# lllyasviel/stable-diffusion-webui-forge

Hardware: AMD Instinct MI355X
Metric: sampler it/s (UNet steps/sec) (higher is better)
Workload: dtype f16; 1 GPU; SDXL UNet 1024x1024 batch=8/GPU fp16, Euler sampler, CFG 7.0 (network batch 16), HIP-graph replay=on; global_batch=8, parallelism=batch-shard x1 (RCCL broadcast cond + gather latents)

## Files before the change

stable-diffusion-webui-forge_amd/csrc/fmx_attention.hip:

```cpp
#include <stdlib.h>

#include "fmx_common.hpp"

namespace {

struct AttnParams {
  const f16* q;
  const f16* k;
  const f16* vt;
  f16* o;
  long q_bs, q_rs, k_bs, k_rs, vt_bs, vt_hs, vt_ds, o_bs, o_rs;
  int batch, heads, nq, nk, nk_pad, qtiles;
  float scale_log2e;
  int causal;
  const f16* zp;
  unsigned q_span;
  unsigned k_span, vt_span;
  const f16* mask;
  long mask_bs, mask_hs, mask_qs;
  float inv_scale;
  int nfull, nsplit;
  int bid0;
};

// ... 798 lines not shown
  const int wg = xcd_remap(blockIdx.x, p.nfull);
  const int qt = wg % p.qtiles, bh = wg / p.qtiles;
  const int h = bh % p.heads, b = bh / p.heads;
  const int q0 = qt * 256 + grp * 64;
  const int ntiles = (p.nk + KVB - 1) / KVB;
  char* const pbase = smem + OFF_P + grp * PSLOT;
  float* const lbase = reinterpret_cast<float*>(smem + OFF_L) + grp * 128;

  if (is_s) {
    const f16* kbase = p.k + (long)b * p.k_bs + (long)h * DP;
    const __amdgpu_buffer_rsrc_t rs_k = __builtin_amdgcn_make_buffer_rsrc(const_cast<f16*>(kbase), 0, p.k_span, 0x00020000);
    unsigned k_voff[NPK];
#pragma unroll
    for (int e = 0; e < NPK; ++e) {
      const int row = (e * 4 + grp) * KROWS + lane / CPR;
      k_voff[e] = (unsigned)row * (unsigned)p.k_rs * 2u + (unsigned)k_logical_chunk<CPR>(row, lane % CPR) * 16u;
    }
    const unsigned k_tile = (unsigned)KVB * (unsigned)p.k_rs * 2u;
    auto stage_k = [&](int slot, int kt) __attribute__((always_inline)) {
#pragma unroll
      for (int e = 0; e < NPK; ++e) {
        auto* dk = (__attribute__((address_space(3))) void*)(smem + slot * KBYTES + (e * 4 + grp) * 1024);
        const unsigned kv = k_voff[e];
        __builtin_amdgcn_raw_ptr_buffer_load_lds(rs_k, dk, 16, kv, (unsigned)kt * k_tile, 0, 0);
      }
    };
    stage_k(0, 0);
    if (ntiles > 1) stage_k(1, 1);
    const float c2 = p.scale_log2e;
    f16x8 qf[2][DSTEPS];
#pragma unroll
    for (int a = 0; a < 2; ++a) {
      const int qrow = min(q0 + a * 32 + li, p.nq - 1);
      const f16* qp = p.q + (long)b * p.q_bs + (long)qrow * p.q_rs + (long)h * DP + hi * 8;
#pragma unroll
      for (int ds = 0; ds < DSTEPS; ++ds) {
        const f16x8 raw = *reinterpret_cast<const f16x8*>(qp + ds * 16);
#pragma unroll
        for (int e = 0; e < 8; ++e) qf[a][ds][e] = (f16)((float)raw[e] * c2);
      }
    }
    float m_run[2] = {0.f, 0.f}, l_run[2] = {0.f, 0.f};
    f16x8 ones, mfrag[2];
#pragma unroll
    for (int e = 0; e < 8; ++e) {
      ones[e] = (f16)((hi == 0 && e < 2) ? 1.0f : 0.0f);
      mfrag[0][e] = mfrag[1][e] = (f16)0.0f;
    }
    const int krow = key_perm(li);
    wait_vmcnt0();
    __builtin_amdgcn_s_barrier();
    typedef unsigned u32x2 __attribute__((ext_vector_type(2)));
    f32x16 sacc[2][2];
    f16x8 kf[2][DSTEPS];
    auto read_k = [&](int which, const char* sk, int half) __attribute__((always_inline)) {
#pragma unroll
      for (int ds = 0; ds < DSTEPS; ++ds) {
        const int row = half * 32 + krow;
        kf[which][ds] = *reinterpret_cast<const f16x8*>(sk + row * (DP * 2) + (k_phys_chunk<CPR>(row, ds * 2 + hi) << 4));
      }
    };
    auto scores = [&](int which) __attribute__((always_inline)) {
#pragma unroll
      for (int a = 0; a < 2; ++a) {
        f32x16 z;
#pragma unroll
        for (int r = 0; r < 16; ++r) z[r] = 0.f;
        sacc[which][a] = FMX_MFMA_32x32x16(ones, mfrag[a], z);
      }
#pragma unroll
      for (int ds = 0; ds < DSTEPS; ++ds)
#pragma unroll
        for (int a = 0; a < 2; ++a) sacc[which][a] = FMX_MFMA_32x32x16(kf[which][ds], qf[a][ds], sacc[which][a]);
    };
    __builtin_amdgcn_sched_barrier(0);
    read_k(0, smem, 0);
    read_k(1, smem, 1);
    scores(0);
    __builtin_amdgcn_sched_barrier(0);
    int kslot_next = ntiles > 1 ? 1 : 0;
    for (int t = 0; t <= ntiles; ++t) {
      if (t < ntiles) {
        if (t + 2 < ntiles) stage_k(kslot_next == 2 ? 0 : kslot_next + 1, t + 2);
        const char* skn = smem + kslot_next * KBYTES;
        char* const ps = pbase + (t & 1) * (4 * PSLOT);
        float* const ctrl = reinterpret_cast<float*>(ps + 8 * 1024);
        const bool ragged = (t + 1) * KVB > p.nk;
#pragma unroll
        for (int s2 = 0; s2 < 2; ++s2) {
          __builtin_amdgcn_sched_barrier(0);
          if (ragged) {
#pragma unroll
            for (int a = 0; a < 2; ++a)
#pragma unroll
              for (int r = 0; r < 16; ++r)
                if (t * KVB + s2 * 32 + hi * 16 + r >= p.nk) sacc[s2][a][r] = -INFINITY;
          }
          float mx[2];
#pragma unroll
          for (int a = 0; a < 2; ++a) {
            float m0 = fmaxf(sacc[s2][a][0], sacc[s2][a][1]);
#pragma unroll
            for (int r = 2; r < 16; r += 2) m0 = fmaxf(fmaxf(m0, sacc[s2][a][r]), sacc[s2][a][r + 1]);
            const u32x2 sw = __builtin_amdgcn_permlane32_swap(__float_as_uint(m0), __float_as_uint(m0), false, false);
            mx[a] = fmaxf(__uint_as_float(sw[0]), __uint_as_float(sw[1]));
          }
          const bool first = t == 0 && s2 == 0;
          const bool moved = first || __any(fmaxf(mx[0], mx[1]) > (float)THR);
          if (moved) {
#pragma unroll
            for (int a = 0; a < 2; ++a) {
              const float delta = first ? mx[a] : fmaxf(mx[a], 0.f);
              const float alpha = first ? 1.0f : __builtin_amdgcn_exp2f(-delta);
              m_run[a] += delta;
              l_run[a] *= alpha;
              const f16 mh = (f16)(-m_run[a]);
              const f16 ml = (f16)(-m_run[a] - (float)mh);
              mfrag[a][0] = hi == 0 ? mh : (f16)0.0f;
              mfrag[a][1] = hi == 0 ? ml : (f16)0.0f;
              ctrl[(s2 * 2 + a) * 64 + lane] = alpha;
#pragma unroll
              for (int r = 0; r < 16; ++r) sacc[s2][a][r] -= delta;
            }
          }
          if (lane == 0) reinterpret_cast<int*>(ctrl)[256 + s2] = (moved && !first) ? 1 : 0;
          __builtin_amdgcn_sched_barrier(0);
          if (s2 == 0) {
            scores(1);
            read_k(0, skn, 0);
          } else {
            scores(0);
            read_k(1, skn, 1);
          }
#pragma unroll
          for (int a = 0; a < 2; ++a) {
            float ps0 = 0.f, ps1 = 0.f;
            f16x8 pf[2];
#pragma unroll
            for (int r = 0; r < 16; ++r) {
              const float e = __builtin_amdgcn_exp2f(sacc[s2][a][r]);
              if (r & 1) ps1 += e; else ps0 += e;
              pf[r >> 3][r & 7] = (f16)e;
            }
#pragma unroll
            for (int j = 0; j < 2; ++j) *reinterpret_cast<f16x8*>(ps + ((a * 2 + s2) * 2 + j) * 1024 + lane * 16) = pf[j];
            l_run[a] += ps0 + ps1;
          }
#pragma unroll
          for (int i = 0; i < 2 * DSTEPS + 2; ++i) {
            __builtin_amdgcn_sched_group_barrier(0x008, 1, 0);
            if (i < DSTEPS) __builtin_amdgcn_sched_group_barrier(0x100, 1, 0);
            __builtin_amdgcn_sched_group_barrier(0x402, (80 + DSTEPS) / (2 * DSTEPS + 2), 0);
          }
          __builtin_amdgcn_sched_barrier(0);
        }
        if (t + 1 == ntiles) {
          lbase[lane] = l_run[0];
          lbase[64 + lane] = l_run[1];
        }
        kslot_next = kslot_next == 2 ? 0 : kslot_next + 1;
      }
      asm volatile("s_waitcnt vmcnt(0) lgkmcnt(0)" ::: "memory");
      __builtin_amdgcn_s_barrier();
    }
    return;
  }

  const f16* vbase = p.vt + (long)b * p.vt_bs + (long)h * p.vt_hs;
  const __amdgpu_buffer_rsrc_t rs_v = __builtin_amdgcn_make_buffer_rsrc(const_cast<f16*>(vbase), 0, p.vt_span, 0x00020000);
  unsigned v_voff[NPV];
#pragma unroll
  for (int e = 0; e < NPV; ++e) {
    const int row = (e * 4 + grp) * 8 + (lane >> 3);
    v_voff[e] = (unsigned)row * (unsigned)p.vt_ds * 2u + (unsigned)((lane & 7) ^ ((row >> 1) & 7)) * 16u;
  }
  auto stage_v = [&](int slot, int kt) __attribute__((always_inline)) {
#pragma unroll
    for (int e = 0; e < NPV; ++e) {
      auto* dv = (__attribute__((address_space(3))) void*)(smem + OFF_V + slot * VBYTES + (e * 4 + grp) * 1024);
      const unsigned vv = v_voff[e];
      __builtin_amdgcn_raw_ptr_buffer_load_lds(rs_v, dv, 16, vv, (unsigned)kt * (KVB * 2u), 0, 0);
    }
  };
  f32x16 oacc[DVT][2];
#pragma unroll
  for (int a = 0; a < 2; ++a)
#pragma unroll
    for (int r = 0; r < 16; ++r)
#pragma unroll
      for (int i = 0; i < DVT; ++i) oacc[i][a][r] = 0.f;
  wait_vmcnt0();
  __builtin_amdgcn_s_barrier();
  int vslot = 0;
  for (int t = 0; t <= ntiles; ++t) {
    if (t < ntiles) stage_v(t & 1, t);
    if (t >= 1) {
      const int u = t - 1;
      const char* ps = pbase + (u & 1) * (4 * PSLOT);
      const float* ctrl = reinterpret_cast<const float*>(ps + 8 * 1024);
      const char* sv = smem + OFF_V + vslot * VBYTES;
      typedef int i32x2 __attribute__((ext_vector_type(2)));
      const i32x2 flags = *reinterpret_cast<const i32x2*>(ctrl + 256);
      f16x8 pf[2][2][2], vf[2][DVT][2];
      auto read_p = [&](int s2) __attribute__((always_inline)) {
#pragma unroll
        for (int a = 0; a < 2; ++a)
#pragma unroll
          for (int j = 0; j < 2; ++j) pf[s2][a][j] = *reinterpret_cast<const f16x8*>(ps + ((a * 2 + s2) * 2 + j) * 1024 + lane * 16);
      };
      auto read_v = [&](int s2, int dt) __attribute__((always_inline)) {
        const int row = dt * 32 + li;
        const char* rp = sv + row * 128;
        const int sw = (row >> 1) & 7;
#pragma unroll
        for (int j = 0; j < 2; ++j) vf[s2][dt][j] = *reinterpret_cast<const f16x8*>(rp + (((s2 * 4 + hi * 2 + j) ^ sw) << 4));
      };
      auto rescale = [&](int s2) __attribute__((always_inline)) {
#pragma unroll
        for (int a = 0; a < 2; ++a) {
          const float alpha = ctrl[(s2 * 2 + a) * 64 + lane];
#pragma unroll
          for (int r = 0; r < 16; ++r)
#pragma unroll
            for (int i = 0; i < DVT; ++i) oacc[i][a][r] *= alpha;
        }
      };
      __builtin_amdgcn_sched_barrier(0);
      read_p(0);
#pragma unroll
      for (int dt = 0; dt < DVT / 2; ++dt) read_v(0, dt);
      __builtin_amdgcn_sched_barrier(0);
      if (flags[0]) rescale(0);
      __builtin_amdgcn_sched_barrier(0);
#pragma unroll
      for (int dt = DVT / 2; dt < DVT; ++dt) read_v(0, dt);
      read_p(1);
#pragma unroll
      for (int dt = 0; dt < DVT / 2; ++dt) read_v(1, dt);
#pragma unroll
      for (int dt = 0; dt < DVT; ++dt)
#pragma unroll
        for (int j = 0; j < 2; ++j)
#pragma unroll
          for (int a = 0; a < 2; ++a) oacc[dt][a] = FMX_MFMA_32x32x16(vf[0][dt][j], pf[0][a][j], oacc[dt][a]);
#pragma unroll
      for (int i = 0; i < 4; ++i) {
        __builtin_amdgcn_sched_group_barrier(0x008, 2, 0);
        __builtin_amdgcn_sched_group_barrier(0x100, 2, 0);
      }
#pragma unroll
      for (int i = 4; i < 2 * DVT; ++i) {
        __builtin_amdgcn_sched_group_barrier(0x008, 2, 0);
        __builtin_amdgcn_sched_group_barrier(0x100, 1, 0);
      }
      __builtin_amdgcn_sched_barrier(0);
      if (flags[1]) rescale(1);
      __builtin_amdgcn_sched_barrier(0);
#pragma unroll
      for (int dt = DVT / 2; dt < DVT; ++dt) read_v(1, dt);
#pragma unroll
      for (int dt = 0; dt < DVT; ++dt)
#pragma unroll
        for (int j = 0; j < 2; ++j)
#pragma unroll
          for (int a = 0; a < 2; ++a) oacc[dt][a] = FMX_MFMA_32x32x16(vf[1][dt][j], pf[1][a][j], oacc[dt][a]);
#pragma unroll
      for (int i = 0; i < DVT; ++i) {
        __builtin_amdgcn_sched_group_barrier(0x008, 2, 0);
        __builtin_amdgcn_sched_group_barrier(0x100, 1, 0);
      }
      __builtin_amdgcn_sched_barrier(0);
    }
    vslot = t & 1;
    asm volatile("s_waitcnt vmcnt(0) lgkmcnt(0)" ::: "memory");
    __builtin_amdgcn_s_barrier();
  }
  typedef unsigned u32x2 __attribute__((ext_vector_type(2)));
#pragma unroll
  for (int a = 0; a < 2; ++a) {
    const float lr = lbase[a * 64 + lane];
    const u32x2 lw = __builtin_amdgcn_permlane32_swap(__float_as_uint(lr), __float_as_uint(lr), false, false);
    const float inv = 1.0f / (__uint_as_float(lw[0]) + __uint_as_float(lw[1]));
    const int qg = q0 + a * 32 + li;
    f16* op = p.o + (long)b * p.o_bs + (long)qg * p.o_rs + (long)h * DP;
#pragma unroll
    for (int dt = 0; dt < DVT; ++dt)
#pragma unroll
      for (int g = 0; g < 4; g += 2) {
        union { f16x4 h4; unsigned u[2]; } lo, up;
#pragma unroll
        for (int e = 0; e < 4; ++e) {
          lo.h4[e] = (f16)(oacc[dt][a][g * 4 + e] * inv);
          up.h4[e] = (f16)(oacc[dt][a][(g + 1) * 4 + e] * inv);
        }
        const u32x2 x = __builtin_amdgcn_permlane32_swap(lo.u[0], up.u[0], false, false);
        const u32x2 y = __builtin_amdgcn_permlane32_swap(lo.u[1], up.u[1], false, false);
        typedef unsigned u32x4 __attribute__((ext_vector_type(4)));
        const u32x4 v = {x[0], y[0], x[1], y[1]};
        if (qg < p.nq) *reinterpret_cast<u32x4*>(op + dt * 32 + (g + hi) * 8) = v;
      }
  }
}

template <int NB>
__global__ __launch_bounds__(256, 2) void attn_short2_kernel(const AttnParams p) {
  extern __shared__ __attribute__((aligned(16))) char smem[];
  constexpr int DP = 64, DSTEPS = 4, CPR = 8;
  constexpr int KBYTES = KVB * DP * 2;
  constexpr int STAGE = KBYTES + 2 * 32 * 128;
  constexpr int NT = (NB + 1) / 2;
  constexpr int KV_BYTES = 2 * STAGE;

  const int tid = threadIdx.x, lane = tid & 63;
  const int wave = __builtin_amdgcn_readfirstlane(tid >> 6);
  const int hi = lane >> 5, li = lane & 31;
  char* const slots = smem + KV_BYTES + wave * 8192;
  const int total = p.batch * p.heads * p.qtiles;
  const int per = (total + (int)gridDim.x - 1) / (int)gridDim.x;
  const int wg = xcd_remap(blockIdx.x, gridDim.x);
  const int g0 = wg * per, g1 = min(total, g0 + per);
  if (g0 >= g1) return;

  const float c2 = p.scale_log2e;
  const int krow = key_perm(li);
  const int r8 = lane >> 3, pc = lane & 7;
  typedef unsigned u32x2 __attribute__((ext_vector_type(2)));
  typedef unsigned u32x4 __attribute__((ext_vector_type(4)));

  int bh_cur = -1;
  __amdgpu_buffer_rsrc_t rs_q = __builtin_amdgcn_make_buffer_rsrc(const_cast<f16*>(p.q), 0, 0, 0x00020000);
  auto q_desc = [&](int bh) {
    const int h = bh % p.heads, b = bh / p.heads;
    return __builtin_amdgcn_make_buffer_rsrc(const_cast<f16*>(p.q + (long)b * p.q_bs + (long)h * DP), 0, p.q_span, 0x00020000);
  };
  auto dma_q = [&](const __amdgpu_buffer_rsrc_t& rs, int tile, int slot) {
#pragma unroll
    for (int e = 0; e < 4; ++e) {
      const int row = e * 8 + r8;
      const unsigned off = (unsigned)(tile * 128 + wave * 32 + row) * (unsigned)p.q_rs * 2u + (unsigned)k_logical_chunk<CPR>(row, pc) * 16u;
      auto* dst = (__attribute__((address_space(3))) void*)(slots + slot * 4096 + e * 1024);
      __builtin_amdgcn_raw_ptr_buffer_load_lds(rs, dst, 16, off, 0, 0, 0);
    }
  };

  int slot = 0;
  for (int g = g0; g < g1; ++g) {
    const int bh = g / p.qtiles, tile = g - bh * p.qtiles;
    const int h = bh % p.heads, b = bh / p.heads;
    if (bh != bh_cur) {
      if (bh_cur >= 0) {
        wait_vmcnt0();
        __syncthreads();
      }
      bh_cur = bh;
      rs_q = q_desc(bh);
      const f16* kbase = p.k + (long)b * p.k_bs + (long)h * DP;
      const f16* vbase = p.vt + (long)b * p.vt_bs + (long)h * p.vt_hs;
      const __amdgpu_buffer_rsrc_t rs_k = __builtin_amdgcn_make_buffer_rsrc(const_cast<f16*>(kbase), 0, p.k_span, 0x00020000);
      const __amdgpu_buffer_rsrc_t rs_v = __builtin_amdgcn_make_buffer_rsrc(const_cast<f16*>(vbase), 0, p.vt_span, 0x00020000);
#pragma unroll
      for (int kt = 0; kt < NT; ++kt)
#pragma unroll
        for (int e = 0; e < 2; ++e) {
          const int kr = (e * 4 + wave) * 8 + lane / CPR;
          const unsigned kv = (unsigned)kr * (unsigned)p.k_rs * 2u + (unsigned)k_logical_chunk<CPR>(kr, lane % CPR) * 16u;
          auto* dk = (__attribute__((address_space(3))) void*)(smem + kt * STAGE + (e * 4 + wave) * 1024);
          __builtin_amdgcn_raw_ptr_buffer_load_lds(rs_k, dk, 16, kv, (unsigned)kt * ((unsigned)KVB * (unsigned)p.k_rs * 2u), 0, 0);
          const int vr = (e * 4 + wave) * 8 + (lane >> 3);
          const unsigned vv = (unsigned)vr * (unsigned)p.vt_ds * 2u + (unsigned)((lane & 7) ^ ((vr >> 1) & 7)) * 16u;
          auto* dv = (__attribute__((address_space(3))) void*)(smem + kt * STAGE + KBYTES + (e * 4 + wave) * 1024);
          __builtin_amdgcn_raw_ptr_buffer_load_lds(rs_v, dv, 16, vv, (unsigned)kt * (KVB * 2u), 0, 0);
        }
      dma_q(rs_q, tile, slot);
      wait_vmcnt0();
      __syncthreads();
    } else {
      asm volatile("s_waitcnt vmcnt(4)" ::: "memory");
    }
    f16x8 qf[DSTEPS];
    {
      const char* qs = slots + slot * 4096 + li * 128;
#pragma unroll
      for (int ds = 0; ds < DSTEPS; ++ds) {
        const f16x8 raw = *reinterpret_cast<const f16x8*>(qs + (k_phys_chunk<CPR>(li, ds * 2 + hi) << 4));
#pragma unroll
        for (int e = 0; e < 8; ++e) qf[ds][e] = (f16)((float)raw[e] * c2);
      }
    }
    const bool more = g + 1 < g1 && (g + 1) / p.qtiles == bh;
    asm volatile("" ::: "memory");
    __builtin_amdgcn_sched_barrier(0);
    if (more) dma_q(rs_q, tile + 1, slot ^ 1);
    __builtin_amdgcn_sched_barrier(0);
    asm volatile("" ::: "memory");

    f32x16 sacc[NB];
#pragma unroll
    for (int gk = 0; gk < NB; ++gk) {
#pragma unroll
      for (int r = 0; r < 16; ++r) sacc[gk][r] = 0.f;
      const char* sk = smem + (gk >> 1) * STAGE;
      const int row = (gk & 1) * 32 + krow;
#pragma unroll
      for (int ds = 0; ds < DSTEPS; ++ds) {
        const f16x8 kf = *reinterpret_cast<const f16x8*>(sk + row * (DP * 2) + (k_phys_chunk<CPR>(row, ds * 2 + hi) << 4));
        sacc[gk] = FMX_MFMA_32x32x16(kf, qf[ds], sacc[gk]);
      }
      __builtin_amdgcn_sched_barrier(0);
    }
#pragma unroll
    for (int gk = 0; gk < NB; ++gk)
      if ((gk + 1) * 32 > p.nk) {
#pragma unroll
        for (int r = 0; r < 16; ++r)
          if (gk * 32 + hi * 16 + r >= p.nk) sacc[gk][r] = -INFINITY;
      }
    float m0 = sacc[0][0];
#pragma unroll
    for (int gk = 0; gk < NB; ++gk)
#pragma unroll
      for (int r = 0; r < 16; ++r) m0 = fmaxf(m0, sacc[gk][r]);
    const u32x2 sw = __builtin_amdgcn_permlane32_swap(__float_as_uint(m0), __float_as_uint(m0), false, false);
    const float mx = fmaxf(__uint_as_float(sw[0]), __uint_as_float(sw[1]));
    float l = 0.f;
    f16x8 pf[NB][2];
#pragma unroll
    for (int gk = 0; gk < NB; ++gk)
#pragma unroll
      for (int r = 0; r < 16; ++r) {
        const float e = __builtin_amdgcn_exp2f(sacc[gk][r] - mx);
        l += e;
        pf[gk][r >> 3][r & 7] = (f16)e;
      }
    f32x16 oacc[2];
#pragma unroll
    for (int dt = 0; dt < 2; ++dt) {
#pragma unroll
      for (int r = 0; r < 16; ++r) oacc[dt][r] = 0.f;
      const int row = dt * 32 + li;
      const int swz = (row >> 1) & 7;
#pragma unroll
      for (int gk = 0; gk < NB; ++gk) {
        const char* rp = smem + (gk >> 1) * STAGE + KBYTES + row * 128;
#pragma unroll
        for (int j = 0; j < 2; ++j) {
          const f16x8 vf = *reinterpret_cast<const f16x8*>(rp + ((((gk & 1) * 4 + hi * 2 + j) ^ swz) << 4));
          oacc[dt] = FMX_MFMA_32x32x16(vf, pf[gk][j], oacc[dt]);
        }
      }
      __builtin_amdgcn_sched_barrier(0);
    }
    const u32x2 lw = __builtin_amdgcn_permlane32_swap(__float_as_uint(l), __float_as_uint(l), false, false);
    const float inv = 1.0f / (__uint_as_float(lw[0]) + __uint_as_float(lw[1]));
    char* os = slots + slot * 4096;
#pragma unroll
    for (int dt = 0; dt < 2; ++dt)
#pragma unroll
      for (int gq = 0; gq < 4; gq += 2) {
        union { f16x4 h4; unsigned u[2]; } lo, up;
#pragma unroll
        for (int e = 0; e < 4; ++e) {
          lo.h4[e] = (f16)(oacc[dt][gq * 4 + e] * inv);
          up.h4[e] = (f16)(oacc[dt][(gq + 1) * 4 + e] * inv);
        }
        const u32x2 x = __builtin_amdgcn_permlane32_swap(lo.u[0], up.u[0], false, false);
        const u32x2 y = __builtin_amdgcn_permlane32_swap(lo.u[1], up.u[1], false, false);
        const u32x4 v = {x[0], y[0], x[1], y[1]};
        const int chunk = dt * 4 + gq + hi;
        *reinterpret_cast<u32x4*>(os + li * 128 + (k_phys_chunk<CPR>(li, chunk) << 4)) = v;
      }
    f16* obase = p.o + (long)b * p.o_bs + (long)h * DP;
#pragma unroll
    for (int e = 0; e < 4; ++e) {
      const int row = e * 8 + r8;
      const u32x4 v = *reinterpret_cast<const u32x4*>(os + row * 128 + (pc << 4));
      const int qg = tile * 128 + wave * 32 + row;
      if (qg < p.nq) *reinterpret_cast<u32x4*>(obase + (long)qg * p.o_rs + k_logical_chunk<CPR>(row, pc) * 8) = v;
    }
    slot ^= 1;
  }
}

struct AttnConfig {
  int cus;
  int allow_split;
  int v3;
};

const AttnConfig& attn_config() {
  static const AttnConfig cfg = [] {
    AttnConfig c{256, 1, 1};
    int dev = 0, cus = 0;
    if (hipGetDevice(&dev) == hipSuccess && hipDeviceGetAttribute(&cus, hipDeviceAttributeMultiprocessorCount, dev) == hipSuccess && cus > 0) c.cus = cus;
    if (const char* e = fmx_knob("FMX_ATTN_SPLIT")) c.allow_split = atoi(e);
    if (const char* e = fmx_knob("FMX_ATTN_V3")) c.v3 = atoi(e);
    return c;
  }();
  return cfg;
}

enum AttnKernel { ATTN_GENERIC, ATTN_SHORT2, ATTN_Q64V3, ATTN_Q64V2, ATTN_WS };

struct AttnLaunch {
  AttnKernel kernel;
  int grid, block, lds;
  int nfull, nsplit, bid0;
};

struct AttnPlan {
  AttnLaunch main, tail;
  int qtiles;
  unsigned q_span, k_span, vt_span;
};

constexpr int attn_stage_bytes(int dp) { return KVB * dp * 2 + (dp + 31) / 32 * 32 * 128; }
constexpr int SHORT2_LDS = 2 * attn_stage_bytes(64) + 4 * 8192;
constexpr int attn_ws_lds(int dp) { return 3 * KVB * dp * 2 + 2 * (dp / 32) * 32 * 128 + 2 * 4 * (8 * 1024 + 1280) + 2048; }

AttnPlan attn_plan(const AttnParams& p, int dp, bool force32, const AttnConfig& cfg) {
  const int smem = 2 * attn_stage_bytes(dp);
  AttnPlan generic{};
  generic.qtiles = (p.nq + 127) / 128;
  generic.main = {ATTN_GENERIC, generic.qtiles * p.heads * p.batch, 256, smem, 0, 0, 0};
  if ((dp != 64 && dp != 128) || p.nq < 256 || force32 || p.causal || p.mask) return generic;
  const double k_span = ((double)(p.nk_pad - 1) * p.k_rs + dp) * 2.0, v_span = ((dp - 1.0) * p.vt_ds + p.nk_pad) * 2.0;
  if (!(k_span < 2.0e9 && v_span < 2.0e9 && p.k_rs > 0 && p.vt_ds > 0)) return generic;
  AttnPlan pl{};
  pl.k_span = (unsigned)k_span;
  pl.vt_span = (unsigned)v_span;
  pl.qtiles = (p.nq + 255) / 256;
  const int grid = pl.qtiles * p.heads * p.batch;
  const int slots = (dp == 64 ? 2 : 1) * cfg.cus;
  const int ntiles = (p.nk + KVB - 1) / KVB;
  const int rem = grid % slots;
  const bool do_split = cfg.allow_split && rem > 0 && 8 * rem <= 3 * slots && ntiles >= 4 && (ntiles & 1) == 0;
  if (dp == 128 && (!do_split || grid > slots)) {
    const int nfull = do_split ? grid - rem : grid;
    pl.main = {ATTN_WS, nfull, 512, attn_ws_lds(dp), nfull, 0, 0};
    if (do_split) pl.tail = {ATTN_Q64V2, 2 * rem, 256, 2 * smem, nfull, 2 * rem, nfull};
    return pl;
  }
  if (dp == 64 && p.nk <= 128) {
    pl.qtiles = (p.nq + 127) / 128;
    const long total = (long)p.batch * p.heads * pl.qtiles;
    const double q_span = ((double)(p.nq - 1) * p.q_rs + 64) * 2.0;
    if (q_span >= 2.0e9 || total >= (1L << 30)) return generic;
    pl.q_span = (unsigned)q_span;
    pl.main = {ATTN_SHORT2, (int)(total < 2 * cfg.cus ? total : 2 * cfg.cus), 256, SHORT2_LDS, 0, 0, 0};
    return pl;
  }
  if (dp == 64 && !do_split && (cfg.v3 == 2 || (cfg.v3 == 1 && ntiles <= 4))) {
    pl.main = {ATTN_Q64V3, grid, 256, 3 * smem / 2, grid, 0, 0};
    return pl;
  }
  const int nfull = do_split ? grid - rem : grid, nsplit = do_split ? 2 * rem : 0;
  pl.main = {ATTN_Q64V2, nfull + nsplit, 256, do_split ? 2 * smem : smem, nfull, nsplit, 0};
  return pl;
}

template <void (*KERNEL)(AttnParams), int MAX_LDS>
int launch_attn_kernel(const AttnLaunch& l, AttnParams p, hipStream_t st, const char* what) {
  static const hipError_t attr = hipFuncSetAttribute(reinterpret_cast<const void*>(KERNEL), hipFuncAttributeMaxDynamicSharedMemorySize, MAX_LDS);
  (void)attr;
  p.nfull = l.nfull;
  p.nsplit = l.nsplit;
  p.bid0 = l.bid0;
  hipLaunchKernelGGL(KERNEL, dim3(l.grid), dim3(l.block), l.lds, st, p);
  FMX_LAUNCH_CHECK(what);
  return FMX_OK;
}

template <int DP>
int launch_attn_plan(AttnParams p, const AttnPlan& pl, hipStream_t st) {
  constexpr int SMEM = 2 * attn_stage_bytes(DP);
  p.qtiles = pl.qtiles;
  p.q_span = pl.q_span;
  p.k_span = pl.k_span;
  p.vt_span = pl.vt_span;
  const AttnLaunch& l = pl.main;
  if (l.kernel == ATTN_GENERIC) return launch_attn_kernel<attn_kernel<DP>, SMEM>(l, p, st, "fmx_attention_f16");
  if constexpr (DP == 64) {
    if (l.kernel == ATTN_SHORT2) {
      const char* what = "fmx_attention_f16 (short context, line-staged)";
      switch ((p.nk + 31) / 32) {
        case 1: return launch_attn_kernel<attn_short2_kernel<1>, SHORT2_LDS>(l, p, st, what);
        case 2: return launch_attn_kernel<attn_short2_kernel<2>, SHORT2_LDS>(l, p, st, what);
        case 3: return launch_attn_kernel<attn_short2_kernel<3>, SHORT2_LDS>(l, p, st, what);
        default: return launch_attn_kernel<attn_short2_kernel<4>, SHORT2_LDS>(l, p, st, what);
      }
    }
    if (l.kernel == ATTN_Q64V3) return launch_attn_kernel<attn_q64v3_kernel<6>, 3 * SMEM / 2>(l, p, st, "fmx_attention_f16 (sub-tile pipelined)");
  }
  if constexpr (DP == 128) {
    if (l.kernel == ATTN_WS) {
      const int rc = launch_attn_kernel<attn_ws_kernel<6, DP>, attn_ws_lds(DP)>(l, p, st, "fmx_attention_f16 (wave-specialised)");
      if (rc != FMX_OK || pl.tail.grid == 0) return rc;
      return launch_attn_kernel<attn_q64v2_kernel<6, DP>, 2 * SMEM>(pl.tail, p, st, "fmx_attention_f16 (key-split tail)");
    }
  }
  if constexpr (DP == 64 || DP == 128) {
    if (l.kernel == ATTN_Q64V2) return launch_attn_kernel<attn_q64v2_kernel<6, DP>, 2 * SMEM>(l, p, st, "fmx_attention_f16 (64 queries per wave)");
  }
  return fmx_set_error(FMX_E_UNSUPPORTED, "attention: no kernel %d at d_head %d", (int)l.kernel, DP);
}

int attn_params(const fmx_attn_args* a, AttnParams& p, bool& force32) {
  FMX_REQUIRE(a && a->q && a->k && a->vt && a->o && a->zero_page, "attention: null pointer");
  FMX_REQUIRE(a->batch > 0 && a->heads > 0 && a->nq > 0 && a->nk > 0, "attention: bad dims");
  FMX_REQUIRE(a->nk_pad >= a->nk && (a->nk_pad % 64) == 0, "attention: nk_pad (%d) must be a multiple of 64 >= nk (%d)", a->nk_pad, a->nk);
  FMX_REQUIRE(fmx_aligned16(a->q) && fmx_aligned16(a->k) && fmx_aligned16(a->vt) && fmx_aligned16(a->o), "attention: 16-byte alignment");
  FMX_REQUIRE((a->q_rs % 8) == 0 && (a->k_rs % 8) == 0 && (a->vt_ds % 8) == 0 && (a->o_rs % 4) == 0 && (a->q_bs % 8) == 0 &&
                  (a->k_bs % 8) == 0 && (a->vt_bs % 8) == 0 && (a->vt_hs % 8) == 0, "attention: strides must be multiples of 8 elements");
  p.q = (const f16*)a->q; p.k = (const f16*)a->k; p.vt = (const f16*)a->vt; p.o = (f16*)a->o;
  p.q_bs = a->q_bs; p.q_rs = a->q_rs; p.k_bs = a->k_bs; p.k_rs = a->k_rs;
  p.vt_bs = a->vt_bs; p.vt_hs = a->vt_hs; p.vt_ds = a->vt_ds; p.o_bs = a->o_bs; p.o_rs = a->o_rs;
  p.batch = a->batch; p.heads = a->heads; p.nq = a->nq; p.nk = a->nk; p.nk_pad = a->nk_pad;
  p.qtiles = 0;
  force32 = a->scale < 0.f;
  p.scale_log2e = fabsf(a->scale) * 1.44269504088896340736f;
  p.zp = (const f16*)a->zero_page;
  p.causal = a->causal ? 1 : 0;
  p.k_span = p.vt_span = p.q_span = 0;
  p.nfull = p.nsplit = p.bid0 = 0;
  p.mask = (const f16*)a->mask; p.mask_bs = a->mask_bs; p.mask_hs = a->mask_hs; p.mask_qs = a->mask_qs;
  p.inv_scale = 1.0f / fabsf(a->scale);
  FMX_REQUIRE(!p.mask || (fmx_aligned16(p.mask) && (p.mask_bs % 8) == 0 && (p.mask_hs % 8) == 0 && (p.mask_qs % 8) == 0),
              "attention: mask must be 16-byte aligned with strides that are multiples of 8 elements (rows padded to nk_pad keys)");
  FMX_REQUIRE(!p.causal || a->nq == a->nk, "attention: the causal mask is defined for self-attention (nq == nk)");
  if (a->dpad != 48 && a->dpad != 64 && a->dpad != 80 && a->dpad != 128 && a->dpad != 160)
    return fmx_set_error(FMX_E_UNSUPPORTED, "attention: dpad %d not in {48,64,80,128,160}", a->dpad);
  return FMX_OK;
}

__global__ void softmax_rows_kernel(f16* __restrict__ x, int ncols, long ld) {
  __shared__ float red[8];
  f16* row = x + (long)blockIdx.x * ld;
  const int tid = threadIdx.x, lane = tid & 63, wave = tid >> 6;
  float mx = -INFINITY;
  for (int j = tid; j < ncols; j += blockDim.x) mx = fmaxf(mx, (float)row[j]);
  mx = wave_max(mx);
  if (lane == 0) red[wave] = mx;
  __syncthreads();
  mx = red[0];
  for (int i = 1; i < (int)(blockDim.x >> 6); ++i) mx = fmaxf(mx, red[i]);
  __syncthreads();
  float sum = 0.f;
  for (int j = tid; j < ncols; j += blockDim.x) sum += __expf((float)row[j] - mx);
  sum = wave_sum(sum);
  if (lane == 0) red[wave] = sum;
  __syncthreads();
  sum = 0.f;
  for (int i = 0; i < (int)(blockDim.x >> 6); ++i) sum += red[i];
  const float inv = 1.0f / sum;
  for (int j = tid; j < ncols; j += blockDim.x) row[j] = (f16)(__expf((float)row[j] - mx) * inv);
}

}

extern "C" int fmx_attention_f16(const fmx_attn_args* a, void* stream) {
  AttnParams p;
  bool force32;
  if (const int rc = attn_params(a, p, force32)) return rc;
  const AttnPlan pl = attn_plan(p, a->dpad, force32, attn_config());
  hipStream_t st = (hipStream_t)stream;
  switch (a->dpad) {
    case 48: return launch_attn_plan<48>(p, pl, st);
    case 64: return launch_attn_plan<64>(p, pl, st);
    case 80: return launch_attn_plan<80>(p, pl, st);
    case 128: return launch_attn_plan<128>(p, pl, st);
    case 160: return launch_attn_plan<160>(p, pl, st);
    default: return fmx_set_error(FMX_E_UNSUPPORTED, "attention: dpad %d not in {48,64,80,128,160}", a->dpad);
  }
}

#ifndef FMX_ELEM_BF16
extern "C" int fmx_attention_route(const fmx_attn_args* a, int32_t cus, char* buf, int32_t cap) {
  AttnParams p;
  bool force32;
  if (const int rc = attn_params(a, p, force32)) return rc;
  FMX_REQUIRE(cus > 0 && buf && cap > 0, "attention_route: bad args");
  const AttnPlan pl = attn_plan(p, a->dpad, force32, AttnConfig{cus, 1, 1});
  const AttnLaunch& l = pl.main;
  int n = 0;
  switch (l.kernel) {
    case ATTN_GENERIC: n = snprintf(buf, cap, "generic"); break;
    case ATTN_SHORT2: n = snprintf(buf, cap, "short2<%d>", (p.nk + 31) / 32); break;
    case ATTN_Q64V3: n = snprintf(buf, cap, "q64v3"); break;
    case ATTN_Q64V2: n = snprintf(buf, cap, "q64v2<%d> %s", a->dpad, l.nsplit == 0 ? "whole" : l.nfull == 0 ? "split" : "whole+split"); break;
    case ATTN_WS: n = snprintf(buf, cap, "ws<%d>%s", a->dpad, pl.tail.grid ? "+split tail" : ""); break;
  }
  FMX_REQUIRE(n > 0 && n < cap, "attention_route: the name needs %d bytes", n + 1);
  return FMX_OK;
}
#endif

extern "C" int fmx_softmax_rows_f16(void* x, int64_t nrows, int32_t ncols, int64_t ld, void* stream) {
  FMX_REQUIRE(x && nrows > 0 && ncols > 0 && ld >= ncols, "softmax_rows: bad args");
  FMX_REQUIRE(nrows < (1LL << 31), "softmax_rows: too many rows");
  hipLaunchKernelGGL(softmax_rows_kernel, dim3((unsigned)nrows), dim3(256), 0, (hipStream_t)stream, (f16*)x, ncols, (long)ld);
  FMX_LAUNCH_CHECK("fmx_softmax_rows_f16");
  return FMX_OK;
}
```

Measured before the change: 9.827 it/s.

## Add single-slot short attention variant for four workgroups per CU, balance tile split

```diff
diff --git a/stable-diffusion-webui-forge_amd/csrc/fmx_attention.hip b/stable-diffusion-webui-forge_amd/csrc/fmx_attention.hip
--- a/stable-diffusion-webui-forge_amd/csrc/fmx_attention.hip
+++ b/stable-diffusion-webui-forge_amd/csrc/fmx_attention.hip
@@ -1124,23 +1124,28 @@
   }
 }
 
-template <int NB>
-__global__ __launch_bounds__(256, 2) void attn_short2_kernel(const AttnParams p) {
+template <int NB, int SLOTS>
+__global__ __launch_bounds__(256) __attribute__((amdgpu_waves_per_eu(SLOTS == 1 ? 4 : 2, 4))) void attn_short2_kernel(const AttnParams p) {
   extern __shared__ __attribute__((aligned(16))) char smem[];
   constexpr int DP = 64, DSTEPS = 4, CPR = 8;
   constexpr int KBYTES = KVB * DP * 2;
   constexpr int STAGE = KBYTES + 2 * 32 * 128;
   constexpr int NT = (NB + 1) / 2;
-  constexpr int KV_BYTES = 2 * STAGE;
+  constexpr bool ODD = SLOTS == 1 && (NB & 1) != 0;
+  constexpr int KV_BYTES = SLOTS == 1 ? NB * (STAGE / 2) : 2 * STAGE;
 
   const int tid = threadIdx.x, lane = tid & 63;
   const int wave = __builtin_amdgcn_readfirstlane(tid >> 6);
   const int hi = lane >> 5, li = lane & 31;
-  char* const slots = smem + KV_BYTES + wave * 8192;
+  char* const slots = smem + KV_BYTES + wave * (SLOTS * 4096);
   const int total = p.batch * p.heads * p.qtiles;
-  const int per = (total + (int)gridDim.x - 1) / (int)gridDim.x;
-  const int wg = xcd_remap(blockIdx.x, gridDim.x);
-  const int g0 = wg * per, g1 = min(total, g0 + per);
+  const int nwg = (int)gridDim.x;
+  const int per = total / nwg, rem = total - per * nwg;
+  const int wg = xcd_remap(blockIdx.x, nwg);
+  const int xcd = (int)blockIdx.x & 7, kx = (int)blockIdx.x >> 3;
+  const int ex = (rem >> 3) + (xcd < (rem & 7) ? 1 : 0);
+  const int g0 = wg * per + (rem >> 3) * xcd + min(xcd, rem & 7) + min(kx, ex);
+  const int g1 = g0 + per + (kx < ex ? 1 : 0);
   if (g0 >= g1) return;
 
   const float c2 = p.scale_log2e;
@@ -1181,23 +1186,38 @@
       const __amdgpu_buffer_rsrc_t rs_k = __builtin_amdgcn_make_buffer_rsrc(const_cast<f16*>(kbase), 0, p.k_span, 0x00020000);
       const __amdgpu_buffer_rsrc_t rs_v = __builtin_amdgcn_make_buffer_rsrc(const_cast<f16*>(vbase), 0, p.vt_span, 0x00020000);
 #pragma unroll
-      for (int kt = 0; kt < NT; ++kt)
-#pragma unroll
-        for (int e = 0; e < 2; ++e) {
-          const int kr = (e * 4 + wave) * 8 + lane / CPR;
+      for (int kt = 0; kt < NT; ++kt) {
+        const unsigned k_tile = (unsigned)kt * ((unsigned)KVB * (unsigned)p.k_rs * 2u), v_tile = (unsigned)kt * (KVB * 2u);
+        if (ODD && kt == NT - 1) {
+          const int kr = wave * 8 + lane / CPR;
           const unsigned kv = (unsigned)kr * (unsigned)p.k_rs * 2u + (unsigned)k_logical_chunk<CPR>(kr, lane % CPR) * 16u;
-          auto* dk = (__attribute__((address_space(3))) void*)(smem + kt * STAGE + (e * 4 + wave) * 1024);
-          __builtin_amdgcn_raw_ptr_buffer_load_lds(rs_k, dk, 16, kv, (unsigned)kt * ((unsigned)KVB * (unsigned)p.k_rs * 2u), 0, 0);
-          const int vr = (e * 4 + wave) * 8 + (lane >> 3);
-          const unsigned vv = (unsigned)vr * (unsigned)p.vt_ds * 2u + (unsigned)((lane & 7) ^ ((vr >> 1) & 7)) * 16u;
-          auto* dv = (__attribute__((address_space(3))) void*)(smem + kt * STAGE + KBYTES + (e * 4 + wave) * 1024);
-          __builtin_amdgcn_raw_ptr_buffer_load_lds(rs_v, dv, 16, vv, (unsigned)kt * (KVB * 2u), 0, 0);
+          auto* dk = (__attribute__((address_space(3))) void*)(smem + kt * STAGE + wave * 1024);
+          __builtin_amdgcn_raw_ptr_buffer_load_lds(rs_k, dk, 16, kv, k_tile, 0, 0);
+          const int vr = wave * 16 + (lane >> 2);
+          const unsigned vv = (unsigned)vr * (unsigned)p.vt_ds * 2u + (unsigned)((lane & 3) ^ ((vr >> 2) & 3)) * 16u;
+          auto* dv = (__attribute__((address_space(3))) void*)(smem + kt * STAGE + KBYTES / 2 + wave * 1024);
+          __builtin_amdgcn_raw_ptr_buffer_load_lds(rs_v, dv, 16, vv, v_tile, 0, 0);
+        } else {
+#pragma unroll
+          for (int e = 0; e < 2; ++e) {
+            const int kr = (e * 4 + wave) * 8 + lane / CPR;
+            const unsigned kv = (unsigned)kr * (unsigned)p.k_rs * 2u + (unsigned)k_logical_chunk<CPR>(kr, lane % CPR) * 16u;
+            auto* dk = (__attribute__((address_space(3))) void*)(smem + kt * STAGE + (e * 4 + wave) * 1024);
+            __builtin_amdgcn_raw_ptr_buffer_load_lds(rs_k, dk, 16, kv, k_tile, 0, 0);
+            const int vr = (e * 4 + wave) * 8 + (lane >> 3);
+            const unsigned vv = (unsigned)vr * (unsigned)p.vt_ds * 2u + (unsigned)((lane & 7) ^ ((vr >> 1) & 7)) * 16u;
+            auto* dv = (__attribute__((address_space(3))) void*)(smem + kt * STAGE + KBYTES + (e * 4 + wave) * 1024);
+            __builtin_amdgcn_raw_ptr_buffer_load_lds(rs_v, dv, 16, vv, v_tile, 0, 0);
+          }
         }
+      }
       dma_q(rs_q, tile, slot);
       wait_vmcnt0();
       __syncthreads();
+    } else if constexpr (SLOTS == 2) {
+      asm volatile("s_waitcnt vmcnt(4)" ::: "memory");
     } else {
-      asm volatile("s_waitcnt vmcnt(4)" ::: "memory");
+      wait_vmcnt0();
     }
     f16x8 qf[DSTEPS];
     {
@@ -1210,11 +1230,13 @@
       }
     }
     const bool more = g + 1 < g1 && (g + 1) / p.qtiles == bh;
-    asm volatile("" ::: "memory");
-    __builtin_amdgcn_sched_barrier(0);
-    if (more) dma_q(rs_q, tile + 1, slot ^ 1);
-    __builtin_amdgcn_sched_barrier(0);
-    asm volatile("" ::: "memory");
+    if constexpr (SLOTS == 2) {
+      asm volatile("" ::: "memory");
+      __builtin_amdgcn_sched_barrier(0);
+      if (more) dma_q(rs_q, tile + 1, slot ^ 1);
+      __builtin_amdgcn_sched_barrier(0);
+      asm volatile("" ::: "memory");
+    }
 
     f32x16 sacc[NB];
 #pragma unroll
@@ -1260,10 +1282,11 @@
 #pragma unroll
       for (int r = 0; r < 16; ++r) oacc[dt][r] = 0.f;
       const int row = dt * 32 + li;
-      const int swz = (row >> 1) & 7;
 #pragma unroll
       for (int gk = 0; gk < NB; ++gk) {
-        const char* rp = smem + (gk >> 1) * STAGE + KBYTES + row * 128;
+        const bool half = ODD && gk == NB - 1;
+        const char* rp = smem + (gk >> 1) * STAGE + (half ? KBYTES / 2 + row * 64 : KBYTES + row * 128);
+        const int swz = half ? (row >> 2) & 3 : (row >> 1) & 7;
 #pragma unroll
         for (int j = 0; j < 2; ++j) {
           const f16x8 vf = *reinterpret_cast<const f16x8*>(rp + ((((gk & 1) * 4 + hi * 2 + j) ^ swz) << 4));
@@ -1299,7 +1322,15 @@
       const int qg = tile * 128 + wave * 32 + row;
       if (qg < p.nq) *reinterpret_cast<u32x4*>(obase + (long)qg * p.o_rs + k_logical_chunk<CPR>(row, pc) * 8) = v;
     }
-    slot ^= 1;
+    if constexpr (SLOTS == 2) {
+      slot ^= 1;
+    } else {
+      asm volatile("s_waitcnt lgkmcnt(0)" ::: "memory");
+      __builtin_amdgcn_sched_barrier(0);
+      if (more) dma_q(rs_q, tile + 1, 0);
+      __builtin_amdgcn_sched_barrier(0);
+      asm volatile("" ::: "memory");
+    }
   }
 }
 
@@ -1307,11 +1338,12 @@
   int cus;
   int allow_split;
   int v3;
+  int short_wg;
 };
 
 const AttnConfig& attn_config() {
   static const AttnConfig cfg = [] {
-    AttnConfig c{256, 1, 1};
+    AttnConfig c{256, 1, 1, 2};
     int dev = 0, cus = 0;
     if (hipGetDevice(&dev) == hipSuccess && hipDeviceGetAttribute(&cus, hipDeviceAttributeMultiprocessorCount, dev) == hipSuccess && cus > 0) c.cus = cus;
     if (const char* e = fmx_knob("FMX_ATTN_SPLIT")) c.allow_split = atoi(e);
@@ -1327,6 +1359,7 @@
   AttnKernel kernel;
   int grid, block, lds;
   int nfull, nsplit, bid0;
+  int slots;
 };
 
 struct AttnPlan {
@@ -1336,7 +1369,9 @@
 };
 
 constexpr int attn_stage_bytes(int dp) { return KVB * dp * 2 + (dp + 31) / 32 * 32 * 128; }
-constexpr int SHORT2_LDS = 2 * attn_stage_bytes(64) + 4 * 8192;
+constexpr int LDS_PER_CU = 160 * 1024;
+constexpr int short2_lds(int nb, int slots) { return slots == 2 ? 2 * attn_stage_bytes(64) + 4 * 8192 : nb * (attn_stage_bytes(64) / 2) + 4 * 4096; }
+constexpr int short2_wgs_per_cu(int nb, int slots) { return slots == 2 ? 2 : (LDS_PER_CU / short2_lds(nb, 1) < 4 ? LDS_PER_CU / short2_lds(nb, 1) : 4); }
 constexpr int attn_ws_lds(int dp) { return 3 * KVB * dp * 2 + 2 * (dp / 32) * 32 * 128 + 2 * 4 * (8 * 1024 + 1280) + 2048; }
 
 AttnPlan attn_plan(const AttnParams& p, int dp, bool force32, const AttnConfig& cfg) {
@@ -1368,7 +1403,9 @@
     const double q_span = ((double)(p.nq - 1) * p.q_rs + 64) * 2.0;
     if (q_span >= 2.0e9 || total >= (1L << 30)) return generic;
     pl.q_span = (unsigned)q_span;
-    pl.main = {ATTN_SHORT2, (int)(total < 2 * cfg.cus ? total : 2 * cfg.cus), 256, SHORT2_LDS, 0, 0, 0};
+    const int nb = (p.nk + 31) / 32, slots = cfg.short_wg == 2 ? 2 : 1;
+    const long resident = (long)short2_wgs_per_cu(nb, slots) * cfg.cus;
+    pl.main = {ATTN_SHORT2, (int)(total < resident ? total : resident), 256, short2_lds(nb, slots), 0, 0, 0, slots};
     return pl;
   }
   if (dp == 64 && !do_split && (cfg.v3 == 2 || (cfg.v3 == 1 && ntiles <= 4))) {
@@ -1404,11 +1441,18 @@
   if constexpr (DP == 64) {
     if (l.kernel == ATTN_SHORT2) {
       const char* what = "fmx_attention_f16 (short context, line-staged)";
-      switch ((p.nk + 31) / 32) {
-        case 1: return launch_attn_kernel<attn_short2_kernel<1>, SHORT2_LDS>(l, p, st, what);
-        case 2: return launch_attn_kernel<attn_short2_kernel<2>, SHORT2_LDS>(l, p, st, what);
-        case 3: return launch_attn_kernel<attn_short2_kernel<3>, SHORT2_LDS>(l, p, st, what);
-        default: return launch_attn_kernel<attn_short2_kernel<4>, SHORT2_LDS>(l, p, st, what);
+      const int nb = (p.nk + 31) / 32;
+      if (l.slots == 2) switch (nb) {
+        case 1: return launch_attn_kernel<attn_short2_kernel<1, 2>, short2_lds(1, 2)>(l, p, st, what);
+        case 2: return launch_attn_kernel<attn_short2_kernel<2, 2>, short2_lds(2, 2)>(l, p, st, what);
+        case 3: return launch_attn_kernel<attn_short2_kernel<3, 2>, short2_lds(3, 2)>(l, p, st, what);
+        default: return launch_attn_kernel<attn_short2_kernel<4, 2>, short2_lds(4, 2)>(l, p, st, what);
+      }
+      switch (nb) {
+        case 1: return launch_attn_kernel<attn_short2_kernel<1, 1>, short2_lds(1, 1)>(l, p, st, what);
+        case 2: return launch_attn_kernel<attn_short2_kernel<2, 1>, short2_lds(2, 1)>(l, p, st, what);
+        case 3: return launch_attn_kernel<attn_short2_kernel<3, 1>, short2_lds(3, 1)>(l, p, st, what);
+        default: return launch_attn_kernel<attn_short2_kernel<4, 1>, short2_lds(4, 1)>(l, p, st, what);
       }
     }
     if (l.kernel == ATTN_Q64V3) return launch_attn_kernel<attn_q64v3_kernel<6>, 3 * SMEM / 2>(l, p, st, "fmx_attention_f16 (sub-tile pipelined)");
@@ -1483,7 +1527,10 @@
   AttnParams p;
   bool force32;
   if (const int rc = attn_params(a, p, force32)) return rc;
-  const AttnPlan pl = attn_plan(p, a->dpad, force32, attn_config());
+  AttnConfig cfg = attn_config();
+  if (a->dpad == 64 && a->nk <= 128)
+    if (const char* e = fmx_knob("FMX_ATTN_SHORT_WG")) cfg.short_wg = atoi(e) == 4 ? 4 : 2;
+  const AttnPlan pl = attn_plan(p, a->dpad, force32, cfg);
   hipStream_t st = (hipStream_t)stream;
   switch (a->dpad) {
     case 48: return launch_attn_plan<48>(p, pl, st);
@@ -1501,7 +1548,7 @@
   bool force32;
   if (const int rc = attn_params(a, p, force32)) return rc;
   FMX_REQUIRE(cus > 0 && buf && cap > 0, "attention_route: bad args");
-  const AttnPlan pl = attn_plan(p, a->dpad, force32, AttnConfig{cus, 1, 1});
+  const AttnPlan pl = attn_plan(p, a->dpad, force32, AttnConfig{cus, 1, 1, 2});
   const AttnLaunch& l = pl.main;
   int n = 0;
   switch (l.kernel) {
```

Result: no change. 9.858 it/s, median of 2 (+0.3%).
